# mengcaopku/DCNet

Hardware: AMD Instinct MI355X
Metric: clips/sec (T=8, 416x416, bs8) fwd+bwd (higher is better)
Workload: dtype f32; 1 GPU; T=8 416x416 bs8/GPU L=20 fp32, 64 img/GPU/step as pairs, fwd+5 losses+bwd+RMSprop; arith=f16x2-split MFMA, fp32 accumulate, parallelism=dp1, ranks_seen=1, reducer=none, step=hipGraph replay (fwd+losses+bwd+RMSprop), sampler=mt

## Files before the change

### dcnet_amd/csrc/conv3.hip

```cpp
#include "igemm.h"
#include "prof.h"
#include <type_traits>

namespace {

typedef _Float16 f16x8_t __attribute__((ext_vector_type(8)));
typedef _Float16 f16x4_t __attribute__((ext_vector_type(4)));
constexpr unsigned OOB3 = 0x80000000u;

__device__ __forceinline__ f32x4 ld16(__amdgpu_buffer_rsrc_t r, unsigned voff, unsigned soff) {
  return __builtin_bit_cast(f32x4, __builtin_amdgcn_raw_buffer_load_b128(r, voff, soff, 0));
}
__device__ __forceinline__ __amdgpu_buffer_rsrc_t rsrc3(const float* base, long long bytes) {
  const unsigned n = bytes > 0x7FFFFFF0LL ? 0x7FFFFFF0u : (bytes < 0 ? 0u : (unsigned)bytes);
  return __builtin_amdgcn_make_buffer_rsrc((void*)base, 0, n, 0x00020000);
}
__device__ __forceinline__ float pow2_scale3(unsigned amax_bits) {
  const int be = (int)((amax_bits >> 23) & 0xFF);
  if (be == 0 || be == 255) return 1.f;
  int e = 14 - (be - 126);
  e = e > 100 ? 100 : (e < -100 ? -100 : e);
  return __uint_as_float((unsigned)(e + 127) << 23);
}
__device__ __forceinline__ int row32(int pos, int half) { return pos * 32 + (((half ^ (pos >> 3)) & 1) << 4); }
// ... 430 lines not shown
#pragma unroll
    for (int r = 0; r < 16; ++r) {
      const int m = m0 + wm * 64 + mi * 32 + (r & 3) + 8 * (r >> 2) + 4 * half;
      if (m >= M) continue;
#pragma unroll
      for (int ni = 0; ni < 2; ++ni) {
        if (co_[ni] >= p.Co) continue;
        float v = acc[mi][ni][r] * sc[ni] + sh2[ni];
        if (p.act == DCN_ACT_LEAKY) v = v > 0.f ? v : v * p.slope;
        if (p.residual) v += p.residual[(size_t)m * p.ldr + co_[ni]];
        gout[(size_t)m * p.ldo + co_[ni]] = v;
        vmax = fmaxf(vmax, fabsf(v));
      }
    }
  if (p.amax_out) {
    vmax = wave_max(vmax);
    if (lane == 0) amax_update(p.amax_out, vmax, blockIdx.x * (WM * WN) + wave);
  }
}

DCN_KNOB(g_conv3, "3x3strip", 1, "conv3.hip: 3x3 stride-1 layers on the strip kernel (0 = implicit-GEMM tile)");
DCN_KNOB(g_conv3_bm, "3bm", 0, "conv3.hip: force the strip kernel's M tile (128 | 256; 0 = automatic)");
DCN_KNOB(g_conv3_abl, "3abl", 0, "conv3.hip: timing ablations of the strip kernel, bits (results WRONG)", nullptr, "-DC3_ABL=1", C3_ABL != 0);
DCN_KNOB(g_conv3_m16, "3m16", 1, "conv3.hip: conv3x.hip (16x16x32 MFMAs) for the launches that take the 256-row tile (0 = never; 2 = every strip launch it fits)");

template <int WM, int WN, int A_LD, int NP = 2, int ABL = 0, int LS = 0, bool IN16 = false, bool O32 = false>
int launch3(const IgemmParams& p, int gran, hipStream_t stream) {
  constexpr int NT = 64 * WM * WN, BM = 64 * WM, BN = 64 * WN;
  const int S = BM + 2 * p.Wi + 2;
  const size_t lds = (size_t)2 * NP * (S + 2) * 32 + (size_t)2 * 3 * (NP * BN * 32 + 128);
  static DcnPerDeviceFlag attr_once;
  if (attr_once.first()) {
    (void)hipFuncSetAttribute(reinterpret_cast<const void*>(&conv3_kernel<WM, WN, A_LD, NP, ABL, LS, IN16, O32>), hipFuncAttributeMaxDynamicSharedMemorySize, 160 * 1024);
  }
  const int gm = cdiv(p.M, BM), gn = cdiv(p.Co, BN);
  const double k_alg = 9.0 * p.Ci;
  const double alg_bytes = IN16 ? 2.0 * ((double)p.N * p.Hi * p.Wi * p.Ci + (double)p.Co * k_alg) +
                                      ((O32 ? 4.0 : 2.0) * (1.0 + (p.accumulate ? 1.0 : 0.0)) + (p.residual ? 2.0 : 0.0) + (p.bt_y ? 2.0 : 0.0)) * (double)p.M * p.Co
                                : 4.0 * ((double)p.N * p.Hi * p.Wi * p.Ci + (double)p.Co * k_alg + (double)p.M * p.Co * epilogue_reads(p));
  const int pid = prof_begin(IN16 ? 50 : (NP == 1 ? 33 : (WM == 4 ? 28 : 29)), 2.0 * (double)p.M * p.Co * k_alg, stream, alg_bytes);
  hipLaunchKernelGGL((conv3_kernel<WM, WN, A_LD, NP, ABL, LS, IN16, O32>), dim3(gm * gn), dim3(NT), lds, stream, p, S, gran);
  prof_end(pid, stream);
  DCN_CHECK_LAUNCH("conv3");
  return DCN_OK;
}

constexpr int A_LD_MAX = 4;
// ... 74 lines not shown
  }
  if (seen != 0x1FF) return false;
  const int bm = conv3b_bm(p.M, p.Co, p.Wi);
  if (!bm) return false;
  const int S = bm + 2 * p.Wi + 2;
  return (long long)S * p.ldi * 2 < 0x7FFFFFF0LL && (long long)p.Co * p.ldw * 2 < 0x7FFFFFF0LL;
}
int conv3b_launch(const IgemmParams& p0, int out_f32, hipStream_t stream) {
  IgemmParams p = p0;
  p.wt16 = p0.wt;
  const int bm = conv3b_bm(p.M, p.Co, p.Wi);
  const int S = bm + 2 * p.Wi + 2, need = cdiv(2 * S, 2 * bm);
  if (bm == 128) {
    if (need <= 2) return out_f32 ? launch3<2, 2, 2, 1, 0, 1, true, true>(p, bm, stream) : launch3<2, 2, 2, 1, 0, 1, true, false>(p, bm, stream);
    return out_f32 ? launch3<2, 2, 4, 1, 0, 1, true, true>(p, bm, stream) : launch3<2, 2, 4, 1, 0, 1, true, false>(p, bm, stream);
  }
  if (need <= 2) return out_f32 ? launch3<4, 2, 2, 1, 0, 1, true, true>(p, bm, stream) : launch3<4, 2, 2, 1, 0, 1, true, false>(p, bm, stream);
  return out_f32 ? launch3<4, 2, 4, 1, 0, 1, true, true>(p, bm, stream) : launch3<4, 2, 4, 1, 0, 1, true, false>(p, bm, stream);
}

int conv3_launch(const IgemmParams& p, int gran, hipStream_t stream) {
  int a_need; const int wmm = conv3_tile(p, gran, &a_need);
  if (g_conv3_m16 && !g_conv3_abl && conv3x_takes(p, gran)) {
    const long long wgs = (long long)cdiv(p.M, 256) * cdiv(p.Co, 128);
    const int cus = dcn_device_cus() > 0 ? dcn_device_cus() : 256;
    const bool short_tail = wgs > cus && wgs <= cus + cus / 2;
    if (g_conv3_m16 == 2 || !short_tail) return conv3x_launch(p, gran, stream);
  }
  if (wmm == 2) return launch3_ld<2, 2>(p, gran, stream);
  return launch3_ld<4, 2>(p, gran, stream);
}
```

### dcnet_amd/csrc/conv3x.hip

```cpp
#include "igemm.h"
#include "prof.h"
#include <type_traits>

namespace {

typedef _Float16 f16x8_t __attribute__((ext_vector_type(8)));
typedef _Float16 f16x4_t __attribute__((ext_vector_type(4)));
constexpr unsigned OOBX = 0x80000000u;

constexpr int XBM = 256, XBN = 128, XNT = 512, XWM = 4;
constexpr int XPB = XBN * 32;
constexpr int XPB1 = XPB + 64;
constexpr int XSLOT = 2 * XPB + 128;
constexpr int XSTAGE = 6 * XSLOT;
constexpr int XA_LD = 4;
#ifndef C3X_ABL
#define C3X_ABL 0
#endif
constexpr int XSMAX = 466;
constexpr int XPA = (XSMAX + 2) * 32;

__device__ __forceinline__ f32x4 ldx16(__amdgpu_buffer_rsrc_t r, unsigned voff, unsigned soff) {
  return __builtin_bit_cast(f32x4, __builtin_amdgcn_raw_buffer_load_b128(r, voff, soff, 0));
}
__device__ __forceinline__ __amdgpu_buffer_rsrc_t rsrcx(const float* base, long long bytes) {
  const unsigned n = bytes > 0x7FFFFFF0LL ? 0x7FFFFFF0u : (bytes < 0 ? 0u : (unsigned)bytes);
  return __builtin_amdgcn_make_buffer_rsrc((void*)base, 0, n, 0x00020000);
}
__device__ __forceinline__ float pow2_scalex(unsigned amax_bits) {
  const int be = (int)((amax_bits >> 23) & 0xFF);
  if (be == 0 || be == 255) return 1.f;
  int e = 14 - (be - 126);
  e = e > 100 ? 100 : (e < -100 ? -100 : e);
  return __uint_as_float((unsigned)(e + 127) << 23);
}

typedef __attribute__((address_space(3))) void lds_voidx;
template <bool DMA>
__global__ __launch_bounds__(XNT, 2) void conv3x_kernel(const IgemmParams p, const int S, const int gran) {
  extern __shared__ __attribute__((aligned(16))) unsigned char smemx[];
  constexpr int PA = XPA;
  unsigned char* const Abase = smemx;
  unsigned char* const Bbase = smemx + 4 * PA;

  const int tid = threadIdx.x, lane = tid & 63, wave = tid >> 6;
  const int wm = wave >> 1, wn = wave & 1;
  const int c16 = lane & 15, g = lane >> 4, tsel = g >> 1, half = g & 1;
  const int gn = (p.Co + XBN - 1) / XBN;
  const int lin = xcd_remap(blockIdx.x, gridDim.x);
  const int bm = lin / gn, bn = lin - bm * gn;
  const int W = p.Wi, H = p.Hi, M = p.M;
  const int m0 = bm * XBM;
  const float sa = pow2_scalex(amax_read(p.amax_a)), sb = p.b_scale[0];

  const int lin0 = m0 - W - 1;
  const int base_px = lin0 > 0 ? lin0 : 0;
  const float* a_base = p.in + (long long)base_px * p.ldi;
  const __amdgpu_buffer_rsrc_t a_rs = rsrcx(a_base, ((long long)(M - base_px - 1) * p.ldi + p.Ci) * 4);
  const __amdgpu_buffer_rsrc_t b_rs = rsrcx(p.wt, (long long)p.Co * p.ldw * 4);

  const int pos0 = tid >> 2, q0 = tid & 3;
  const unsigned a_off0 = (unsigned)((lin0 + pos0 - base_px) * p.ldi * 4 + q0 * 16);
  const int a_st0 = pos0 * 32 + q0 * 8;
  const unsigned a_pstride = (unsigned)(128 * p.ldi * 4);
// ... 8 lines not shown
    unsigned o = a_off0;
    asm volatile("" : "+v"(o));
    return a_ok[j] ? o + (unsigned)j * a_pstride : OOBX;
  };
  auto a_st = [&](const int j) {
    int o = a_st0;
    asm volatile("" : "+v"(o));
    return a_in[j] ? o + j * 4096 : (XSMAX + 1) * 32 + q0 * 8;
  };
  unsigned b_off; int b_st;
  if constexpr (DMA) {
    const int plane = wave & 1, rho = 32 * (wave >> 1) + (lane >> 1), kh = lane & 1;
    const int filt = (rho & ~63) + 4 * (rho & 15) + ((rho & 63) >> 4);
    const int co = bn * XBN + filt;
    b_off = co < p.Co ? (unsigned)(co * p.ldw * 4 + (2 * kh + plane) * 16) : OOBX;
    b_st = __builtin_amdgcn_readfirstlane(plane * XPB1 + (wave >> 1) * 1024);
  } else {
    const int rho = tid >> 2, chunk = tid & 3;
    const int filt = (rho & ~63) + 4 * (rho & 15) + ((rho & 63) >> 4);
    const int co = bn * XBN + filt;
    b_off = co < p.Co ? (unsigned)(co * p.ldw * 4 + chunk * 16) : OOBX;
    b_st = (chunk & 1) * XPB1 + rho * 32 + (chunk >> 1) * 16;
  }
  unsigned msk[4];
#pragma unroll
  for (int i = 0; i < 4; ++i) {
    const int m = m0 + wm * 64 + i * 16 + c16;
    unsigned v = 0;
    if (m < M) {
      const int rem = m % (H * W), y = rem / W, x = rem - y * W;
      for (int t = 0; t < 9; ++t)
        if ((unsigned)(y + p.tap_dy[t]) < (unsigned)H && (unsigned)(x + p.tap_dx[t]) < (unsigned)W) v |= 1u << t;
    }
    msk[i] = v;
  }
  const int a_lane0 = (wm * 64 + c16) * 32 + half * 16;
  const int b_lane0 = (wn * 64 + c16) * 32 + half * 16 + tsel * 3 * XSLOT;

  const int nch = p.Ci >> 4;
  const int nper = nch >> 1;
  const int nsi = 3 * nper;

  f32x4 a_reg[XA_LD], b_reg[6];
  const unsigned lds0 = (unsigned)(uintptr_t)(lds_voidx*)smemx;
  auto store_a_piece = [&](const int buf_off, int j) {
    const f32x4 t = a_reg[j] * sa;
    const f16x4_t h = {(_Float16)t[0], (_Float16)t[1], (_Float16)t[2], (_Float16)t[3]};
    const f16x4_t l = {(_Float16)(t[0] - (float)h[0]), (_Float16)(t[1] - (float)h[1]), (_Float16)(t[2] - (float)h[2]),
                       (_Float16)(t[3] - (float)h[3])};
    if constexpr (DMA) {
      const unsigned addr = lds0 + (unsigned)(buf_off + a_st(j));
      asm volatile("ds_write_b64 %0, %1\n\tds_write_b64 %0, %2 offset:%3"
                   :: "v"(addr), "v"(__builtin_bit_cast(unsigned long long, h)), "v"(__builtin_bit_cast(unsigned long long, l)), "n"(XPA));
    } else {
      unsigned char* abuf = Abase + buf_off;
      *reinterpret_cast<uint2*>(abuf + a_st(j)) = __builtin_bit_cast(uint2, h);
      *reinterpret_cast<uint2*>(abuf + PA + a_st(j)) = __builtin_bit_cast(uint2, l);
    }
  };

  f32x4 acc[4][4];
#pragma unroll
  for (int i = 0; i < 4; ++i)
#pragma unroll
    for (int j = 0; j < 4; ++j) acc[i][j] = f32x4{0.f, 0.f, 0.f, 0.f};

  if (tid < 8) {
    const f32x4 z = {0.f, 0.f, 0.f, 0.f};
    *reinterpret_cast<f32x4*>(Abase + (tid >> 1) * PA + XSMAX * 32 + (tid & 1) * 16) = z;
  }
#pragma unroll
  for (int j = 0; j < XA_LD; ++j) a_reg[j] = ldx16(a_rs, a_off(j), 0u);
  auto dma = [&](const int stage_off, const int slot, const bool live, const unsigned soff) {
    __builtin_amdgcn_raw_ptr_buffer_load_lds(b_rs, (lds_voidx*)(Bbase + stage_off + slot * XSLOT + b_st), 16, (int)(live ? b_off : OOBX),
                                             (int)(live ? soff : 0u), 0, 0);
  };
  if constexpr (DMA) {
#pragma unroll
    for (int q = 0; q < 6; ++q) {
      const int G = q / 3, j = q - 3 * G;
      dma(0, q, true, (unsigned)p.tap_w[3 * G + j] * 4u);
    }
#pragma unroll
    for (int q = 0; q < 2; ++q)
      dma(XSTAGE, q, true, (unsigned)p.tap_w[6 + q] * 4u);
#pragma unroll
// ... 1 lines not shown
#pragma unroll
    for (int j = 0; j < XA_LD; ++j) a_reg[j] = ldx16(a_rs, a_off(j), 64u);
    asm volatile("s_waitcnt vmcnt(0)" ::: "memory");
  } else {
#pragma unroll
    for (int q = 0; q < 6; ++q) {
      const int G = q / 3, j = q - 3 * G;
      b_reg[q] = ldx16(b_rs, b_off, (unsigned)p.tap_w[3 * G + j] * 4u);
    }
#pragma unroll
    for (int j = 0; j < XA_LD; ++j) store_a_piece(0, j);
#pragma unroll
    for (int j = 0; j < XA_LD; ++j) a_reg[j] = ldx16(a_rs, a_off(j), 64u);
#pragma unroll
    for (int q = 0; q < 6; ++q) *reinterpret_cast<f32x4*>(Bbase + q * XSLOT + b_st) = b_reg[q];
#pragma unroll
    for (int q = 0; q < 6; ++q) {
      const int G = q < 3 ? 2 : 0, cc = q < 3 ? 0 : 1, j = q % 3;
      b_reg[q] = ldx16(b_rs, b_off, (unsigned)(p.tap_w[3 * G + j] + cc * 16) * 4u);
    }
  }
  __syncthreads();

  f16x8_t Al[4], Ah[4], Bh[4], Bl[4];
  int ad[4];
  auto a_addr = [&](const int T, const int J) {
    const int Ga = T == 0 ? 0 : (T == 1 ? 2 : 1), Gb = T == 0 ? 1 : (T == 1 ? 0 : 2);
    const int ta = 3 * Ga + J, tb = 3 * Gb + J;
    const int sha = (p.tap_dy[ta] + 1) * W + p.tap_dx[ta] + 1, shb = (p.tap_dy[tb] + 1) * W + p.tap_dx[tb] + 1;
    int ts = tsel;
    asm volatile("" : "+v"(ts));
    const int sh = ts ? shb : sha;
    const int tl = ts ? tb : ta;
    const int bo = T == 0 ? 0 : (T == 2 ? 2 * PA : ts * (2 * PA));
    const int base = bo + a_lane0 + sh * 32;
    const int z = bo + XSMAX * 32;
#pragma unroll
    for (int i = 0; i < 4; ++i) ad[i] = ((msk[i] >> tl) & 1) ? base + i * 512 : z;
  };
  auto read_Al = [&]() {
#pragma unroll
    for (int i = 0; i < 4; ++i) Al[i] = *reinterpret_cast<const f16x8_t*>(Abase + PA + ad[i]);
  };
  auto read_Ah = [&]() {
#pragma unroll
    for (int i = 0; i < 4; ++i) Ah[i] = *reinterpret_cast<const f16x8_t*>(Abase + ad[i]);
  };
  int st_cur = 0;
  auto read_B = [&](f16x8_t (&B)[4], const int stage_off, const int J, const int plane) {
    const unsigned char* bb = Bbase + stage_off + b_lane0;
#pragma unroll
    for (int jn = 0; jn < 4; ++jn) B[jn] = *reinterpret_cast<const f16x8_t*>(bb + J * XSLOT + plane * XPB1 + jn * 512);
  };
  auto mm = [&](const f16x8_t (&A)[4], const f16x8_t (&B)[4]) {
#pragma unroll
    for (int i = 0; i < 4; ++i)
#pragma unroll
      for (int jn = 0; jn < 4; ++jn) acc[i][jn] = __builtin_amdgcn_mfma_f32_16x16x32_f16(A[i], B[jn], acc[i][jn], 0, 0, 0);
  };

  auto body = [&](auto T_, const int u) {
    constexpr int T = decltype(T_)::value;
    constexpr int TN = (T + 1) % 3;
    const int k = 3 * u + T, c0 = 2 * u;
    const bool in_b = k + 2 < nsi;
    const int st_nxt = XSTAGE - st_cur;
    unsigned char* const bw = Bbase + st_nxt + b_st;
    auto side = [&](const int gi) {
      if constexpr (DMA) {
        if (gi < 4 && !(C3X_ABL & 1)) {
          const int sl = gi + 2, second = sl >= 3, j = sl - 3 * second;
          const int G = T == 0 ? (second ? 0 : 2) : (T == 1 ? (second ? 2 : 1) : (second ? 1 : 0));
          const int dc = T == 0 ? (second ? 1 : 0) : (T == 1 ? 1 : 2);
          dma(st_nxt, sl, k + 1 < nsi, (unsigned)(p.tap_w[3 * G + j] + (c0 + dc) * 16) * 4u);
        }
        if (gi >= 7 && !(C3X_ABL & 1)) {
          const int sl = gi - 7;
          const int G = T == 0 ? 1 : (T == 1 ? 0 : 2), dc = T == 0 ? 1 : 2;
          dma(st_cur, sl, in_b, (unsigned)(p.tap_w[3 * G + sl] + (c0 + dc) * 16) * 4u);
// ... 41 lines not shown
      mm(Ah, Bh);
      side(3 * j + 1);
      __builtin_amdgcn_sched_barrier(0);
      if (j < 2) read_B(Bh, st_cur, j + 1, 0); else read_B(Bh, st_nxt, 0, 0);
      __builtin_amdgcn_sched_barrier(0);
      mm(Ah, Bl);
      side(3 * j + 2);
      __builtin_amdgcn_sched_barrier(0);
    }
    st_cur = st_nxt;
  };
  a_addr(0, 0);
  read_Al();
  read_B(Bh, 0, 0, 0);
  {
    using I0 = std::integral_constant<int, 0>; using I1 = std::integral_constant<int, 1>; using I2 = std::integral_constant<int, 2>;
    for (int u = 0; u < nper; ++u) { body(I0{}, u); body(I1{}, u); body(I2{}, u); }
  }
  if constexpr (DMA) asm volatile("s_waitcnt vmcnt(0)" ::: "memory");
  __syncthreads();

  const float dq = 1.f / (sa * sb);
#pragma unroll
  for (int i = 0; i < 4; ++i)
#pragma unroll
    for (int jn = 0; jn < 4; ++jn) acc[i][jn] *= dq;
  const int co0 = bn * XBN + wn * 64 + 4 * c16;
  const bool co_ok = co0 < p.Co;
  const int mrow0 = m0 + wm * 64 + 4 * g;
  float* __restrict__ gout = p.out;
  if (p.accumulate && co_ok) {
#pragma unroll
    for (int i = 0; i < 4; ++i)
#pragma unroll
      for (int r = 0; r < 4; ++r) {
        const int m = mrow0 + 16 * i + r;
        if (m >= M) continue;
        const f32x4 o = *reinterpret_cast<const f32x4*>(gout + (size_t)m * p.ldo + co0);
#pragma unroll
        for (int jn = 0; jn < 4; ++jn) acc[i][jn][r] += o[jn];
      }
  }
  if (p.stats) {
    float* red = reinterpret_cast<float*>(smemx);
    float s[4] = {0.f, 0.f, 0.f, 0.f}, ss[4] = {0.f, 0.f, 0.f, 0.f};
    if (p.bt_y && co_ok) {
      const f32x4 mu = *reinterpret_cast<const f32x4*>(p.bt_mean + co0), is = *reinterpret_cast<const f32x4*>(p.bt_invstd + co0);
      f32x4 ga = {1.f, 1.f, 1.f, 1.f}, be = {0.f, 0.f, 0.f, 0.f};
      if (p.bt_gamma) ga = *reinterpret_cast<const f32x4*>(p.bt_gamma + co0);
      if (p.bt_beta) be = *reinterpret_cast<const f32x4*>(p.bt_beta + co0);
      const float* yb = p.bt_y + co0;
#pragma unroll
      for (int i = 0; i < 4; ++i) {
        f32x4 yv[4];
#pragma unroll
        for (int r = 0; r < 4; ++r) {
          const int m = mrow0 + 16 * i + r;
          yv[r] = *reinterpret_cast<const f32x4*>(yb + (size_t)(m < M ? m : M - 1) * p.Co);
        }
#pragma unroll
        for (int r = 0; r < 4; ++r) {
          const int m = mrow0 + 16 * i + r;
#pragma unroll
          for (int jn = 0; jn < 4; ++jn) {
            const float xh = (yv[r][jn] - mu[jn]) * is[jn];
            float gq = acc[i][jn][r];
            if (p.bt_act == DCN_ACT_LEAKY) gq = (ga[jn] * xh + be[jn] <= 0.f) ? gq * p.bt_slope : gq;
            gq = m < M ? gq : 0.f;
            s[jn] += gq; ss[jn] += gq * xh;
          }
        }
      }
    } else if (!p.bt_y) {
#pragma unroll
      for (int i = 0; i < 4; ++i)
#pragma unroll
        for (int r = 0; r < 4; ++r)
#pragma unroll
          for (int jn = 0; jn < 4; ++jn) { const float v = acc[i][jn][r]; s[jn] += v; ss[jn] = __builtin_fmaf(v, v, ss[jn]); }
    }
#pragma unroll
    for (int jn = 0; jn < 4; ++jn) {
      s[jn] += __shfl_xor(s[jn], 16); ss[jn] += __shfl_xor(ss[jn], 16);
      s[jn] += __shfl_xor(s[jn], 32); ss[jn] += __shfl_xor(ss[jn], 32);
    }
    if (g == 0) {
      const int col = wn * 64 + 4 * c16;
      *reinterpret_cast<f32x4*>(red + (0 * XWM + wm) * XBN + col) = f32x4{s[0], s[1], s[2], s[3]};
      *reinterpret_cast<f32x4*>(red + (1 * XWM + wm) * XBN + col) = f32x4{ss[0], ss[1], ss[2], ss[3]};
    }
    __syncthreads();
    const int groups = XBM / gran, spg = XWM / groups;
    const int rows_total = (M + gran - 1) / gran;
    for (int idx = tid; idx < 2 * XBN * groups; idx += XNT) {
      const int gq = idx / (2 * XBN), rest = idx - gq * 2 * XBN;
      const int which = rest / XBN, col = rest - which * XBN;
      float t = 0.f;
      for (int w = 0; w < spg; ++w) t += red[(which * XWM + gq * spg + w) * XBN + col];
      const int co = bn * XBN + col, srow = bm * groups + gq;
      if (co < p.Co && srow < rows_total) p.stats[((size_t)srow * 2 + which) * p.Co + co] = t;
    }
  }
  float vmax = 0.f;
  if (co_ok) {
    f32x4 sc = {1.f, 1.f, 1.f, 1.f}, sh = {0.f, 0.f, 0.f, 0.f};
    if (p.scale) sc = *reinterpret_cast<const f32x4*>(p.scale + co0);
    if (p.shift) sh = *reinterpret_cast<const f32x4*>(p.shift + co0);
#pragma unroll
    for (int i = 0; i < 4; ++i)
#pragma unroll
      for (int r = 0; r < 4; ++r) {
        const int m = mrow0 + 16 * i + r;
        if (m >= M) continue;
        f32x4 v;
#pragma unroll
        for (int jn = 0; jn < 4; ++jn) {
          float t = acc[i][jn][r] * sc[jn] + sh[jn];
          if (p.act == DCN_ACT_LEAKY) t = t > 0.f ? t : t * p.slope;
          v[jn] = t;
        }
        if (p.residual) v += *reinterpret_cast<const f32x4*>(p.residual + (size_t)m * p.ldr + co0);
        *reinterpret_cast<f32x4*>(gout + (size_t)m * p.ldo + co0) = v;
#pragma unroll
        for (int jn = 0; jn < 4; ++jn) vmax = fmaxf(vmax, fabsf(v[jn]));
      }
  }
  if (p.amax_out) {
    vmax = wave_max(vmax);
    if (lane == 0) amax_update(p.amax_out, vmax, blockIdx.x * 8 + wave);
  }
}

}

bool conv3x_takes(const IgemmParams& p, int gran) {
  if (p.wt16 || (gran != 128 && gran != 256)) return false;
  if (p.Co % 4 != 0 || p.ldo % 4 != 0 || (p.residual && p.ldr % 4 != 0)) return false;
  auto al16 = [](const void* q) { return (reinterpret_cast<uintptr_t>(q) & 15) == 0; };
  if (!al16(p.out) || !al16(p.residual) || !al16(p.bt_y) || !al16(p.scale) || !al16(p.shift) || !al16(p.bt_mean) || !al16(p.bt_invstd) ||
      !al16(p.bt_gamma) || !al16(p.bt_beta)) return false;
  const int S = XBM + 2 * p.Wi + 2;
  if (S > XSMAX) return false;
  return (long long)S * p.ldi * 4 < 0x7FFFFFF0LL && (long long)p.Co * p.ldw * 4 < 0x7FFFFFF0LL;
}

int conv3x_launch(const IgemmParams& p, int gran, hipStream_t stream) {
  const int S = XBM + 2 * p.Wi + 2;
  const size_t lds = (size_t)4 * XPA + (size_t)2 * XSTAGE;
  static_assert((size_t)4 * XPA + (size_t)2 * XSTAGE <= 160 * 1024, "LDS");
  static DcnPerDeviceFlag attr_once;
  if (attr_once.first()) {
    (void)hipFuncSetAttribute(reinterpret_cast<const void*>(&conv3x_kernel<true>), hipFuncAttributeMaxDynamicSharedMemorySize, 160 * 1024);
  }
  const int gm = cdiv(p.M, XBM), gn = cdiv(p.Co, XBN);
  const double k_alg = 9.0 * p.Ci;
  const double alg_bytes = 4.0 * ((double)p.N * p.Hi * p.Wi * p.Ci + (double)p.Co * k_alg + (double)p.M * p.Co * epilogue_reads(p));
  const int pid = prof_begin(51, 2.0 * (double)p.M * p.Co * k_alg, stream, alg_bytes);
  hipLaunchKernelGGL(conv3x_kernel<true>, dim3(gm * gn), dim3(XNT), lds, stream, p, S, gran);
  prof_end(pid, stream);
  DCN_CHECK_LAUNCH("conv3x");
  return DCN_OK;
}
```

### dcnet_amd/csrc/igemm.h

```cpp
#pragma once
#include "common.h"

#define IGEMM_MAX_TAPS 16


struct IgemmParams {
  const float* in;
  const float* wt;
  const float* f8;
  const unsigned* amax_a;
  const unsigned* amax_b;
  const void* wt16;
  const float* b_scale;
  unsigned* amax_out;
  float* out;
  const float* scale;
  const float* shift;
  const float* residual;
  float* stats;
  const float* row_scale;
  int batch;
  long long in_bs, wt_bs, out_bs;
  int bmode;
  int kvalid;
// ... 5 lines not shown
  int Co, ldo, ldr, ldw;
  int M;
  int ntaps;
  int cpt, kiters;
  int act; float slope;
  int accumulate, dense_out, c4;
  int acc_post;
  int tap_dy[IGEMM_MAX_TAPS], tap_dx[IGEMM_MAX_TAPS], tap_w[IGEMM_MAX_TAPS];
  int ncls;
  int cls_M[4], cls_Hs[4], cls_Ws[4], cls_oy0[4], cls_ox0[4], cls_ntaps[4];
  const float* bt_y; const float* bt_mean; const float* bt_invstd; const float* bt_gamma; const float* bt_beta;
  int bt_act; float bt_slope;
  const unsigned char* a_scale8; const unsigned char* b_scale8;
};
inline double epilogue_reads(const IgemmParams& p) { return 1.0 + (p.accumulate ? 1.0 : 0.0) + (p.residual ? 1.0 : 0.0) + (p.bt_y ? 1.0 : 0.0); }
bool igemm_tap_capable(const IgemmParams& p);

int igemm_grid_m(int M, int Co, int ntaps);
int igemm_launch(const IgemmParams& p, hipStream_t stream);
bool igemm_will_presplit(long long rows, int Co, int ntaps, int Ci);

bool conv3_applicable(const IgemmParams& p, int precision, int gran);
int conv3_launch(const IgemmParams& p, int gran, hipStream_t stream);
bool conv3x_takes(const IgemmParams& p, int gran);
int conv3x_launch(const IgemmParams& p, int gran, hipStream_t stream);
int conv3b_bm(int M, int Co, int Wi);
bool conv3b_takes(const IgemmParams& p);
int conv3b_launch(const IgemmParams& p, int out_f32, hipStream_t stream);

bool conv1_applicable(const IgemmParams& p, int precision, int gran);
int conv1_launch(const IgemmParams& p, int gran, hipStream_t stream);
int conv1_tile_of(long long rows, int Co, int ntaps, int Ci, int stats, int gran, int storage16);
int conv1b_grid_m(int M, int Co, int ntaps, int s1_w = 0);
int conv1b_launch(const IgemmParams& p, int out_f32, hipStream_t stream);
int conv1q_grid_m(int M, int Co);
int conv1q_launch(const IgemmParams& p, int out_f32, hipStream_t stream);
bool conv2b_takes(int M, int Co, int ntaps);
int conv2b_launch(const IgemmParams& p, int out_f32, hipStream_t stream);


bool stem_applicable(const IgemmParams& p, const float* scratch);
int stem_launch(const IgemmParams& p, float* scratch, hipStream_t stream);

bool dgrad2_applicable(int n, int h, int wd, int cin, int cout, int ksize, int stride, int accumulate);
struct DcnBnTap { const float* y; const float* mean; const float* invstd; const float* gamma; const float* beta; int act; float slope;
                  float* stats; int stats_rows; };
int nconv1_launch_b16(int mode, const void* x, int ldi, const void* w16, void* y, int ldo, float* stats, int stats_rows,
                      int n, int h, int wd, int stride, hipStream_t stream);
// ... 19 lines not shown
```

### dcnet_amd/lib.py

```python
from __future__ import annotations

import ctypes
import os
from ctypes import c_char_p, c_double, c_float, c_int, c_int64, c_void_p

_HERE = os.path.dirname(os.path.abspath(__file__))
LIB_PATH = os.path.join(_HERE, "libdcnet_hip.so")

P, I, L, F, D = c_void_p, c_int, c_int64, c_float, c_double

SIGNATURES = {
    "dcn_last_error": (c_char_p, []),
    "dcn_version": (I, []),
    "dcn_nchw_to_nhwc": (I, [P, P, I, I, I, I, I, P]),
    "dcn_nhwc_to_nchw": (I, [P, P, I, I, I, I, I, P]),
    "dcn_oihw_to_ohwi": (I, [P, P, I, I, I, I, I, P]),
    "dcn_ohwi_to_oihw": (I, [P, P, I, I, I, I, I, P]),
    "dcn_conv2d_fwd": (I, [P, P, P, I, I, I, I, I, I, I, P, P, I, F, P, I, I, P, I, P, P, P, P, P, I, P]),
    "dcn_absmax": (I, [P, L, I, I, P, P]),
    "dcn_f8_scale": (I, [P, L, I, I, P, P, P]),
    "dcn_conv2d_stats_rows": (I, [I, I, I, I, I, I]),
    "dcn_conv1_tile": (I, [L, I, I, I, I, I]),
    "dcn_l2norm_score_fwd_form": (I, [I]),
    "dcn_bn_apply_form": (I, [I, I]),
    "dcn_igemm_split_build": (I, [I, I]),
    "dcn_gemm3_variant": (I, []),
    "dcn_conv2d_bwd_data": (I, [P, I, P, P, P, I, I, I, I, I, I, I, I, P, P, P, I, P, P]),
    "dcn_conv2d_bwd_data_tap": (I, [P, I, P, P, P, I, I, I, I, I, I, I, I, P, P, P, I, P, P, P, P, P, P, I, F, P, I, P, P]),
    "dcn_conv2d_bwd_data_tap_rows": (I, [I, I, I, I, I, I, I]),
    "dcn_conv2d_pre_supported": (I, [I, I, I, I, I, I, I]),
    "dcn_conv2d_fwd_pre": (I, [P, P, P, I, I, I, I, I, I, I, P, P, I, F, I, P, P, P, P]),
    "dcn_conv2d_bwd_weight_pre_supported": (I, [I, I, I, I, I, I, I]),
    "dcn_conv2d_bwd_weight_pre": (I, [P, I, P, I, P, P, P, I, I, I, I, I, I, I, P, P, I, F, P, P, P]),
    "dcn_bn_act_amax_bound": (I, [P, P, P, I, F, P, P]),
    "dcn_gemm3_supported": (I, [I, I, I, I]),
    "dcn_gemm3_presplit": (I, [P, I, L, P, I, L, I, I, I, P, P]),
    "dcn_gemm3": (I, [P, I, L, I, P, I, L, I, P, I, L, P, L, I, I, I, I, I, P, P, P]),
    "dcn_filter_job_bytes": (I, []),
    "dcn_prepare_filters": (I, [P, I, I, I, P, L, P]),
    "dcn_conv2d_geom_size": (L, [I, I, I, I, I]),
    "dcn_conv2d_geom": (I, [P, I, I, I, I, I, P]),
    "dcn_conv2d_bwd_weight": (I, [P, I, P, I, P, P, P, P, I, I, I, I, I, I, I, P, P, P]),
    "dcn_conv2d_bwd_weight_ws": (L, [I, I, I, I, I, I, I]),
    "dcn_stem_bwd_weight_bn": (I, [P, P, P, I, P, P, P, P, I, F, P, L, I, I, I, I, P, P, P]),
    "dcn_stem_bwd_weight_bn_ws": (L, [I, I, I]),
    "dcn_stem_bwd_weight_bn_b16": (I, [P, P, P, I, P, P, P, P, I, F, P, L, I, I, I, I, P, P, P]),
    "dcn_bn_ws": (L, [I]),
    "dcn_bn_finalize": (I, [P, I, I, L, P, P, F, F, P, P, P, P, P, P, P, P]),
    "dcn_bn_fold": (I, [P, P, P, P, F, I, P, P, P]),
# ... 131 lines not shown
    "dcn_conv2d_fwd_f8": (I, [P, P, P, P, P, I, I, I, I, I, I, I, I, P, P, I, F, P, I, I, P, I, P]),
    "dcn_conv2d_bwd_data_f8": (I, [P, P, P, P, P, I, I, I, I, I, I, I, I, I, P, P, P, P, P, I, F, P, I, P, P]),
    "dcn_post_topk": (I, [P, P, P, P, P, I, I, I, I, P, P, P, P, P, P, P, P, P]),
    "dcn_post_fusion": (I, [P, P, P, P, I, I, I, I, P, P, P]),
    "dcn_clip_prep_ws": (L, [I, I]),
    "dcn_clip_prep": (I, [P, L, P, P, I, I, P, P, P, P]),
    "dcn_bank_write": (I, [P, I, P, P, L, I, P]),
    "dcn_coattn_bank_fwd": (I, [P, P, P, P, L, P, P, I, L, P, P, P, P, I, I, I, F, P]),
    "dcn_post_fusion_bank": (I, [P, P, I, I, I, I, P, P, P]),
    "dcn_bank_write_b16": (I, [P, I, P, P, P, L, I, P]),
    "dcn_bank_concat_b16": (I, [P, L, P, I, L, P, I, I, I, P]),
    "dcn_coattn_bank_form": (I, [I, I]),
    "dcn_post_nms": (I, [P, I, I, F, P, P]),
    "dcn_tube_transitions": (I, [P, P, I, I, I, I, I, I, F, F, P, P]),
    "dcn_tube_forward": (I, [P, P, P, P, I, I, I, I, I, P, P, P]),
    "dcn_tube_backtrack": (I, [P, P, I, I, I, P, P, P]),
    "dcn_tube_stream_step": (I, [P, P, P, I, I, I, I, I, P, P, P, P, P]),
    "dcn_tube_stream_flush": (I, [P, P, I, I, I, I, P, P, P]),
}
_VALUE_FUNCS = {"dcn_version", "dcn_conv2d_stats_rows", "dcn_conv2d_bwd_data_tap_rows", "dcn_conv2d_pre_supported",
                "dcn_conv2d_bwd_weight_pre_supported", "dcn_gemm3_supported", "dcn_channel_stats_rows", "dcn_filter_job_bytes", "dcn_prof_records",
                "dcn_conv2d_stats_rows_b16", "dcn_bn_act_bwd_reduce_rows_b16", "dcn_conv2d_stats_rows_f8", "dcn_quant_fusable", "dcn_quant_job_bytes",
                "dcn_conv1_tile", "dcn_l2norm_score_fwd_form", "dcn_bn_apply_form", "dcn_igemm_split_build", "dcn_gemm3_variant",
                "dcn_coattn_bank_form"}
ABI_VERSION = 318


class DcnError(RuntimeError):
    pass


class _Lib:
    def __init__(self, path: str):
        if not os.path.exists(path):
            raise DcnError(
                f"{path} not found: build it with `python -m dcnet_amd.build` "
                "(hipcc --offload-arch=gfx950).  There is no CPU or eager fallback.")
        self._dll = ctypes.CDLL(path)
        for name, (res, args) in SIGNATURES.items():
            try:
                fn = getattr(self._dll, name)
            except AttributeError as e:
                raise DcnError(f"{path} does not export {name}; rebuild the library") from e
            fn.restype = res
            fn.argtypes = args
            if res is I and name not in _VALUE_FUNCS:
                setattr(self, name[4:], self._checked(name, fn))
# ... 41 lines not shown
```

### include/dcnet_hip.h

```cpp
#ifndef DCNET_HIP_H
#define DCNET_HIP_H

#include <stdint.h>

#ifdef __cplusplus
extern "C" {
#endif

#define DCN_OK 0
#define DCN_ERR_ARG (-1)
#define DCN_ERR_LAUNCH (-2)

#define DCN_AMAX_WORDS 64
#define DCN_SLAB_COUNTERS 4096

#define DCN_ACT_NONE 0
#define DCN_ACT_LEAKY 1

#define DCN_ABI_VERSION 318

const char* dcn_last_error(void);
int dcn_version(void);

int dcn_nchw_to_nhwc(const float* src, float* dst, int n, int c, int h, int w, int c_pad, void* stream);
int dcn_nhwc_to_nchw(const float* src, float* dst, int n, int c, int h, int w, int ld, void* stream);
int dcn_oihw_to_ohwi(const float* src, float* dst, int co, int ci, int kh, int kw, int ci_pad, void* stream);
int dcn_ohwi_to_oihw(const float* src, float* dst, int co, int ci, int kh, int kw, int ci_pad, void* stream);

int dcn_conv2d_fwd(const float* x, const float* w, float* y,
                   int n, int h, int wd, int cin, int cout, int ksize, int stride,
                   const float* scale, const float* shift, int act, float slope,
                   const float* residual, int ldr, int ldy,
                   float* stats, int accumulate, const float* f8_scales,
                   const uint32_t* amax_x, const uint32_t* amax_w, uint32_t* amax_y, float* w_split, int w_split_ready,
                   void* stream);
int dcn_absmax(const float* x, int64_t rows, int c, int ld, uint32_t* amax, void* stream);
int dcn_conv2d_stats_rows(int n, int h, int wd, int cout, int ksize, int stride);
int dcn_conv1_tile(int64_t rows, int cout, int ntaps, int cin, int stats, int storage);
int dcn_l2norm_score_fwd_form(int c);
int dcn_bn_apply_form(int c, int params_aligned);
int dcn_igemm_split_build(int kind, int ksteps);
int dcn_gemm3_variant(void);
int dcn_f8_scale(const float* x, int64_t rows, int c, int ld, float* scale, void* ws, void* stream);

int dcn_conv2d_bwd_data(const float* dy, int lddy, const float* w, float* wt, float* dx,
                        int n, int h, int wd, int cin, int cout, int ksize, int stride,
                        int accumulate, const float* f8_scales, const uint32_t* amax_dy, const uint32_t* amax_w,
                        int wt_ready, const float* wt_split, void* stream);
int dcn_conv2d_bwd_data_tap(const float* dy, int lddy, const float* w, float* wt, float* dx,
                            int n, int h, int wd, int cin, int cout, int ksize, int stride,
                            int accumulate, const float* f8_scales, const uint32_t* amax_dy, const uint32_t* amax_w,
                            int wt_ready, const float* wt_split,
                            const float* tap_y, const float* tap_mean, const float* tap_invstd, const float* tap_gamma,
                            const float* tap_beta, int tap_act, float tap_slope, float* tap_stats, int tap_stats_rows,
                            int* tap_rows, void* stream);
int dcn_conv2d_bwd_data_tap_rows(int n, int h, int wd, int cin, int cout, int ksize, int stride);
int dcn_conv2d_pre_supported(int n, int h, int wd, int cin, int cout, int ksize, int stride);
int dcn_conv2d_fwd_pre(const float* x, const float* w, float* y, int n, int h, int wd, int cin, int cout, int ksize, int stride,
                       const float* pre_scale, const float* pre_shift, int pre_act, float pre_slope,
                       int ldy, float* stats, const uint32_t* amax_x, const uint32_t* amax_w, void* stream);
int dcn_conv2d_bwd_weight_pre_supported(int n, int h, int wd, int cin, int cout, int ksize, int stride);
int dcn_conv2d_bwd_weight_pre(const float* x, int ldx, const float* dy, int lddy, float* dw, float* ws, uint32_t* counters,
                              int n, int h, int wd, int cin, int cout, int ksize, int stride,
                              const float* pre_scale, const float* pre_shift, int pre_act, float pre_slope,
                              const uint32_t* amax_x, const uint32_t* amax_dy, void* stream);
// ... 353 lines not shown
```

Measured before the change: 88.49 clips/s.

## Add 128/192-row tile variants to conv3x and pick tile height by wave quantization

The 16x16x32-MFMA strip kernel is templated on the M tile height (128, 192 or 256 rows), and a cost table picks the height that minimizes rounds of workgroups over the CU count. Grids that previously fell back to the older strip kernel on a short tail can now run conv3x with a smaller tile that fills the last round better. Statistics partials are restricted to tile heights that map onto the slab granularity, and the 128-row tile chains its per-wave sums through LDS. The cost weights are heuristic, so a smaller tile may lose per-tile reuse without gaining enough occupancy.

Result: no change. 88.40 clips/s (-0.1%).

```diff
diff --git a/dcnet_amd/csrc/conv3.hip b/dcnet_amd/csrc/conv3.hip
--- a/dcnet_amd/csrc/conv3.hip
+++ b/dcnet_amd/csrc/conv3.hip
@@ -476,7 +476,7 @@
 DCN_KNOB(g_conv3, "3x3strip", 1, "conv3.hip: 3x3 stride-1 layers on the strip kernel (0 = implicit-GEMM tile)");
 DCN_KNOB(g_conv3_bm, "3bm", 0, "conv3.hip: force the strip kernel's M tile (128 | 256; 0 = automatic)");
 DCN_KNOB(g_conv3_abl, "3abl", 0, "conv3.hip: timing ablations of the strip kernel, bits (results WRONG)", nullptr, "-DC3_ABL=1", C3_ABL != 0);
-DCN_KNOB(g_conv3_m16, "3m16", 1, "conv3.hip: conv3x.hip (16x16x32 MFMAs) for the launches that take the 256-row tile (0 = never; 2 = every strip launch it fits)");
+DCN_KNOB(g_conv3_m16, "3m16", 1, "conv3.hip: conv3x.hip (16x16x32 MFMAs; 1 = 256-row tiles, 192-row tiles where conv3x_pick_bm says so, other grids of 1 to 1.5 rounds of 256-row tiles on conv3.hip; 0 = never; 2 = every strip launch it fits, at that height; 3 = 256-row tiles only, the rule before the tile heights; 128 | 192 | 256 = that tile height forced where the launch's partial rows admit it)");
 
 template <int WM, int WN, int A_LD, int NP = 2, int ABL = 0, int LS = 0, bool IN16 = false, bool O32 = false>
 int launch3(const IgemmParams& p, int gran, hipStream_t stream) {
@@ -597,10 +597,15 @@
 int conv3_launch(const IgemmParams& p, int gran, hipStream_t stream) {
   int a_need; const int wmm = conv3_tile(p, gran, &a_need);
   if (g_conv3_m16 && !g_conv3_abl && conv3x_takes(p, gran)) {
+    const int cus = dcn_device_cus() > 0 ? dcn_device_cus() : 256;
+    const int flags = conv3x_flags(p, gran);
     const long long wgs = (long long)cdiv(p.M, 256) * cdiv(p.Co, 128);
-    const int cus = dcn_device_cus() > 0 ? dcn_device_cus() : 256;
     const bool short_tail = wgs > cus && wgs <= cus + cus / 2;
-    if (g_conv3_m16 == 2 || !short_tail) return conv3x_launch(p, gran, stream);
+    if (g_conv3_m16 == 128 || g_conv3_m16 == 192 || g_conv3_m16 == 256) return conv3x_launch(p, gran, conv3x_fit_bm(g_conv3_m16, flags), stream);
+    const int bm = g_conv3_m16 == 3 ? 256 : conv3x_pick_bm(p.M, p.Co, p.Wi, cus, flags);
+    if (g_conv3_m16 == 2) return conv3x_launch(p, gran, bm, stream);
+    if (bm == 192) return conv3x_launch(p, gran, 192, stream);
+    if (!short_tail) return conv3x_launch(p, gran, 256, stream);
   }
   if (wmm == 2) return launch3_ld<2, 2>(p, gran, stream);
   return launch3_ld<4, 2>(p, gran, stream);
diff --git a/dcnet_amd/csrc/conv3x.hip b/dcnet_amd/csrc/conv3x.hip
--- a/dcnet_amd/csrc/conv3x.hip
+++ b/dcnet_amd/csrc/conv3x.hip
@@ -8,17 +8,21 @@
 typedef _Float16 f16x4_t __attribute__((ext_vector_type(4)));
 constexpr unsigned OOBX = 0x80000000u;
 
-constexpr int XBM = 256, XBN = 128, XNT = 512, XWM = 4;
+constexpr int XBN = 128, XNT = 512, XWM = 4;
+static_assert(XBN == 128 && CONV3X_WMAX == 104, "igemm.h");
+template <int MI> struct XTile {
+  static constexpr int BM = 64 * MI;
+  static constexpr int SMAX = BM + 2 * CONV3X_WMAX + 2;
+  static constexpr int PA = (SMAX + 2) * 32;
+  static constexpr int A_LD = (SMAX + 127) / 128;
+};
 constexpr int XPB = XBN * 32;
 constexpr int XPB1 = XPB + 64;
 constexpr int XSLOT = 2 * XPB + 128;
 constexpr int XSTAGE = 6 * XSLOT;
-constexpr int XA_LD = 4;
 #ifndef C3X_ABL
 #define C3X_ABL 0
 #endif
-constexpr int XSMAX = 466;
-constexpr int XPA = (XSMAX + 2) * 32;
 
 __device__ __forceinline__ f32x4 ldx16(__amdgpu_buffer_rsrc_t r, unsigned voff, unsigned soff) {
   return __builtin_bit_cast(f32x4, __builtin_amdgcn_raw_buffer_load_b128(r, voff, soff, 0));
@@ -36,10 +40,10 @@
 }
 
 typedef __attribute__((address_space(3))) void lds_voidx;
-template <bool DMA>
+template <bool DMA, int MI>
 __global__ __launch_bounds__(XNT, 2) void conv3x_kernel(const IgemmParams p, const int S, const int gran) {
   extern __shared__ __attribute__((aligned(16))) unsigned char smemx[];
-  constexpr int PA = XPA;
+  constexpr int XBM = XTile<MI>::BM, XSMAX = XTile<MI>::SMAX, XPA = XTile<MI>::PA, XA_LD = XTile<MI>::A_LD, PA = XPA;
   unsigned char* const Abase = smemx;
   unsigned char* const Bbase = smemx + 4 * PA;
 
@@ -94,10 +98,10 @@
     b_off = co < p.Co ? (unsigned)(co * p.ldw * 4 + chunk * 16) : OOBX;
     b_st = (chunk & 1) * XPB1 + rho * 32 + (chunk >> 1) * 16;
   }
-  unsigned msk[4];
-#pragma unroll
-  for (int i = 0; i < 4; ++i) {
-    const int m = m0 + wm * 64 + i * 16 + c16;
+  unsigned msk[MI];
+#pragma unroll
+  for (int i = 0; i < MI; ++i) {
+    const int m = m0 + wm * (16 * MI) + i * 16 + c16;
     unsigned v = 0;
     if (m < M) {
       const int rem = m % (H * W), y = rem / W, x = rem - y * W;
@@ -106,7 +110,7 @@
     }
     msk[i] = v;
   }
-  const int a_lane0 = (wm * 64 + c16) * 32 + half * 16;
+  const int a_lane0 = (wm * (16 * MI) + c16) * 32 + half * 16;
   const int b_lane0 = (wn * 64 + c16) * 32 + half * 16 + tsel * 3 * XSLOT;
 
   const int nch = p.Ci >> 4;
@@ -131,9 +135,9 @@
     }
   };
 
-  f32x4 acc[4][4];
-#pragma unroll
-  for (int i = 0; i < 4; ++i)
+  f32x4 acc[MI][4];
+#pragma unroll
+  for (int i = 0; i < MI; ++i)
 #pragma unroll
     for (int j = 0; j < 4; ++j) acc[i][j] = f32x4{0.f, 0.f, 0.f, 0.f};
 
@@ -181,8 +185,8 @@
   }
   __syncthreads();
 
-  f16x8_t Al[4], Ah[4], Bh[4], Bl[4];
-  int ad[4];
+  f16x8_t Al[MI], Ah[MI], Bh[4], Bl[4];
+  int ad[MI];
   auto a_addr = [&](const int T, const int J) {
     const int Ga = T == 0 ? 0 : (T == 1 ? 2 : 1), Gb = T == 0 ? 1 : (T == 1 ? 0 : 2);
     const int ta = 3 * Ga + J, tb = 3 * Gb + J;
@@ -195,15 +199,15 @@
     const int base = bo + a_lane0 + sh * 32;
     const int z = bo + XSMAX * 32;
 #pragma unroll
-    for (int i = 0; i < 4; ++i) ad[i] = ((msk[i] >> tl) & 1) ? base + i * 512 : z;
+    for (int i = 0; i < MI; ++i) ad[i] = ((msk[i] >> tl) & 1) ? base + i * 512 : z;
   };
   auto read_Al = [&]() {
 #pragma unroll
-    for (int i = 0; i < 4; ++i) Al[i] = *reinterpret_cast<const f16x8_t*>(Abase + PA + ad[i]);
+    for (int i = 0; i < MI; ++i) Al[i] = *reinterpret_cast<const f16x8_t*>(Abase + PA + ad[i]);
   };
   auto read_Ah = [&]() {
 #pragma unroll
-    for (int i = 0; i < 4; ++i) Ah[i] = *reinterpret_cast<const f16x8_t*>(Abase + ad[i]);
+    for (int i = 0; i < MI; ++i) Ah[i] = *reinterpret_cast<const f16x8_t*>(Abase + ad[i]);
   };
   int st_cur = 0;
   auto read_B = [&](f16x8_t (&B)[4], const int stage_off, const int J, const int plane) {
@@ -211,9 +215,9 @@
 #pragma unroll
     for (int jn = 0; jn < 4; ++jn) B[jn] = *reinterpret_cast<const f16x8_t*>(bb + J * XSLOT + plane * XPB1 + jn * 512);
   };
-  auto mm = [&](const f16x8_t (&A)[4], const f16x8_t (&B)[4]) {
-#pragma unroll
-    for (int i = 0; i < 4; ++i)
+  auto mm = [&](const f16x8_t (&A)[MI], const f16x8_t (&B)[4]) {
+#pragma unroll
+    for (int i = 0; i < MI; ++i)
 #pragma unroll
       for (int jn = 0; jn < 4; ++jn) acc[i][jn] = __builtin_amdgcn_mfma_f32_16x16x32_f16(A[i], B[jn], acc[i][jn], 0, 0, 0);
   };
@@ -301,16 +305,16 @@
 
   const float dq = 1.f / (sa * sb);
 #pragma unroll
-  for (int i = 0; i < 4; ++i)
+  for (int i = 0; i < MI; ++i)
 #pragma unroll
     for (int jn = 0; jn < 4; ++jn) acc[i][jn] *= dq;
   const int co0 = bn * XBN + wn * 64 + 4 * c16;
   const bool co_ok = co0 < p.Co;
-  const int mrow0 = m0 + wm * 64 + 4 * g;
+  const int mrow0 = m0 + wm * (16 * MI) + 4 * g;
   float* __restrict__ gout = p.out;
   if (p.accumulate && co_ok) {
 #pragma unroll
-    for (int i = 0; i < 4; ++i)
+    for (int i = 0; i < MI; ++i)
 #pragma unroll
       for (int r = 0; r < 4; ++r) {
         const int m = mrow0 + 16 * i + r;
@@ -320,17 +324,17 @@
         for (int jn = 0; jn < 4; ++jn) acc[i][jn][r] += o[jn];
       }
   }
-  if (p.stats) {
+  if constexpr (MI != 3) if (p.stats) {
     float* red = reinterpret_cast<float*>(smemx);
     float s[4] = {0.f, 0.f, 0.f, 0.f}, ss[4] = {0.f, 0.f, 0.f, 0.f};
-    if (p.bt_y && co_ok) {
+    if (MI == 4 && p.bt_y && co_ok) {
       const f32x4 mu = *reinterpret_cast<const f32x4*>(p.bt_mean + co0), is = *reinterpret_cast<const f32x4*>(p.bt_invstd + co0);
       f32x4 ga = {1.f, 1.f, 1.f, 1.f}, be = {0.f, 0.f, 0.f, 0.f};
       if (p.bt_gamma) ga = *reinterpret_cast<const f32x4*>(p.bt_gamma + co0);
       if (p.bt_beta) be = *reinterpret_cast<const f32x4*>(p.bt_beta + co0);
       const float* yb = p.bt_y + co0;
 #pragma unroll
-      for (int i = 0; i < 4; ++i) {
+      for (int i = 0; i < MI; ++i) {
         f32x4 yv[4];
 #pragma unroll
         for (int r = 0; r < 4; ++r) {
@@ -351,25 +355,45 @@
         }
       }
     } else if (!p.bt_y) {
-#pragma unroll
-      for (int i = 0; i < 4; ++i)
-#pragma unroll
-        for (int r = 0; r < 4; ++r)
-#pragma unroll
-          for (int jn = 0; jn < 4; ++jn) { const float v = acc[i][jn][r]; s[jn] += v; ss[jn] = __builtin_fmaf(v, v, ss[jn]); }
+      auto fold = [&]() {
+#pragma unroll
+        for (int i = 0; i < MI; ++i)
+#pragma unroll
+          for (int r = 0; r < 4; ++r)
+#pragma unroll
+            for (int jn = 0; jn < 4; ++jn) { const float v = acc[i][jn][r]; s[jn] += v; ss[jn] = __builtin_fmaf(v, v, ss[jn]); }
+      };
+      if constexpr (MI == 2) {
+        f32x4* chain = reinterpret_cast<f32x4*>(smemx + 2 * XWM * XBN * 4) + (((wm >> 1) * 2 + wn) * 64 + lane) * 2;
+        if (!(wm & 1)) {
+          fold();
+          chain[0] = f32x4{s[0], s[1], s[2], s[3]}; chain[1] = f32x4{ss[0], ss[1], ss[2], ss[3]};
+        }
+        __syncthreads();
+        if (wm & 1) {
+          const f32x4 s0 = chain[0], ss0 = chain[1];
+#pragma unroll
+          for (int jn = 0; jn < 4; ++jn) { s[jn] = s0[jn]; ss[jn] = ss0[jn]; }
+          fold();
+        }
+      } else {
+        fold();
+      }
     }
 #pragma unroll
     for (int jn = 0; jn < 4; ++jn) {
       s[jn] += __shfl_xor(s[jn], 16); ss[jn] += __shfl_xor(ss[jn], 16);
       s[jn] += __shfl_xor(s[jn], 32); ss[jn] += __shfl_xor(ss[jn], 32);
     }
-    if (g == 0) {
+    constexpr int NSL = XBM / 64;
+    const int slab = MI == 2 ? wm >> 1 : wm;
+    if (g == 0 && (MI != 2 || (wm & 1))) {
       const int col = wn * 64 + 4 * c16;
-      *reinterpret_cast<f32x4*>(red + (0 * XWM + wm) * XBN + col) = f32x4{s[0], s[1], s[2], s[3]};
-      *reinterpret_cast<f32x4*>(red + (1 * XWM + wm) * XBN + col) = f32x4{ss[0], ss[1], ss[2], ss[3]};
+      *reinterpret_cast<f32x4*>(red + (0 * XWM + slab) * XBN + col) = f32x4{s[0], s[1], s[2], s[3]};
+      *reinterpret_cast<f32x4*>(red + (1 * XWM + slab) * XBN + col) = f32x4{ss[0], ss[1], ss[2], ss[3]};
     }
     __syncthreads();
-    const int groups = XBM / gran, spg = XWM / groups;
+    const int groups = XBM / gran, spg = NSL / groups;
     const int rows_total = (M + gran - 1) / gran;
     for (int idx = tid; idx < 2 * XBN * groups; idx += XNT) {
       const int gq = idx / (2 * XBN), rest = idx - gq * 2 * XBN;
@@ -386,7 +410,7 @@
     if (p.scale) sc = *reinterpret_cast<const f32x4*>(p.scale + co0);
     if (p.shift) sh = *reinterpret_cast<const f32x4*>(p.shift + co0);
 #pragma unroll
-    for (int i = 0; i < 4; ++i)
+    for (int i = 0; i < MI; ++i)
 #pragma unroll
       for (int r = 0; r < 4; ++r) {
         const int m = mrow0 + 16 * i + r;
@@ -418,25 +442,66 @@
   auto al16 = [](const void* q) { return (reinterpret_cast<uintptr_t>(q) & 15) == 0; };
   if (!al16(p.out) || !al16(p.residual) || !al16(p.bt_y) || !al16(p.scale) || !al16(p.shift) || !al16(p.bt_mean) || !al16(p.bt_invstd) ||
       !al16(p.bt_gamma) || !al16(p.bt_beta)) return false;
-  const int S = XBM + 2 * p.Wi + 2;
-  if (S > XSMAX) return false;
+  if (p.Wi > CONV3X_WMAX) return false;
+  const int S = 256 + 2 * p.Wi + 2;
   return (long long)S * p.ldi * 4 < 0x7FFFFFF0LL && (long long)p.Co * p.ldw * 4 < 0x7FFFFFF0LL;
 }
 
-int conv3x_launch(const IgemmParams& p, int gran, hipStream_t stream) {
-  const int S = XBM + 2 * p.Wi + 2;
-  const size_t lds = (size_t)4 * XPA + (size_t)2 * XSTAGE;
-  static_assert((size_t)4 * XPA + (size_t)2 * XSTAGE <= 160 * 1024, "LDS");
+static const struct { int bm; double cost; } CONV3X_COST[] = {{256, 1.0}, {192, 0.82}, {128, 0.61}};
+
+static bool conv3x_bm_ok(int bm, int flags) {
+  if (!(flags & CONV3X_PARTIALS)) return true;
+  return bm == 256 || (bm == 128 && !(flags & (CONV3X_PARTIALS_256 | CONV3X_TAP)));
+}
+
+int conv3x_pick_bm(int M, int Co, int Wi, int num_cus, int flags) {
+  if (M <= 0 || Co <= 0 || Wi > CONV3X_WMAX) return 0;
+  if (num_cus <= 0) num_cus = 256;
+  const long long gn = cdiv(Co, XBN);
+  int best = 0; double best_t = 0.0;
+  for (const auto& c : CONV3X_COST) {
+    if (!conv3x_bm_ok(c.bm, flags)) continue;
+    const double t = (double)cdiv((long long)cdiv(M, c.bm) * gn, (long long)num_cus) * c.cost;
+    if (!best || t < best_t) { best = c.bm; best_t = t; }
+  }
+  return best;
+}
+int conv3x_fit_bm(int bm, int flags) {
+  if (bm == 192 && !conv3x_bm_ok(192, flags)) bm = 128;
+  if (bm == 128 && !conv3x_bm_ok(128, flags)) bm = 256;
+  return bm == 128 || bm == 192 ? bm : 256;
+}
+
+namespace {
+template <int MI>
+int launch3x(const IgemmParams& p, int gran, hipStream_t stream) {
+  using T = XTile<MI>;
+  const int S = T::BM + 2 * p.Wi + 2;
+  constexpr size_t lds = (size_t)4 * T::PA + (size_t)2 * XSTAGE;
+  static_assert(lds <= 160 * 1024, "LDS");
+  static_assert(2 * XWM * XBN * 4 + 2 * 2 * 64 * 2 * 16 <= lds, "statistics reduction in LDS");
+  static_assert(T::A_LD <= 4 && T::A_LD * 128 >= T::SMAX, "strip pieces");
   static DcnPerDeviceFlag attr_once;
   if (attr_once.first()) {
-    (void)hipFuncSetAttribute(reinterpret_cast<const void*>(&conv3x_kernel<true>), hipFuncAttributeMaxDynamicSharedMemorySize, 160 * 1024);
-  }
-  const int gm = cdiv(p.M, XBM), gn = cdiv(p.Co, XBN);
+    (void)hipFuncSetAttribute(reinterpret_cast<const void*>(&conv3x_kernel<true, MI>), hipFuncAttributeMaxDynamicSharedMemorySize, 160 * 1024);
+  }
+  const int gm = cdiv(p.M, T::BM), gn = cdiv(p.Co, XBN);
   const double k_alg = 9.0 * p.Ci;
   const double alg_bytes = 4.0 * ((double)p.N * p.Hi * p.Wi * p.Ci + (double)p.Co * k_alg + (double)p.M * p.Co * epilogue_reads(p));
   const int pid = prof_begin(51, 2.0 * (double)p.M * p.Co * k_alg, stream, alg_bytes);
-  hipLaunchKernelGGL(conv3x_kernel<true>, dim3(gm * gn), dim3(XNT), lds, stream, p, S, gran);
+  hipLaunchKernelGGL((conv3x_kernel<true, MI>), dim3(gm * gn), dim3(XNT), lds, stream, p, S, gran);
   prof_end(pid, stream);
   DCN_CHECK_LAUNCH("conv3x");
   return DCN_OK;
 }
+}
+
+int conv3x_launch(const IgemmParams& p, int gran, int bm, hipStream_t stream) {
+  DCN_CHECK_ARG(conv3x_bm_ok(bm, conv3x_flags(p, gran)) && p.Wi <= CONV3X_WMAX, "conv3x: a %d-row tile cannot write this launch's partial rows", bm);
+  if (bm == 128) return launch3x<2>(p, gran, stream);
+  if (bm == 192) return launch3x<3>(p, gran, stream);
+  DCN_CHECK_ARG(bm == 256, "conv3x: tile height %d", bm);
+  return launch3x<4>(p, gran, stream);
+}
+
+extern "C" int dcn_conv3x_pick_bm(int m, int cout, int wi, int num_cus, int flags) { return conv3x_pick_bm(m, cout, wi, num_cus, flags); }
diff --git a/dcnet_amd/csrc/igemm.h b/dcnet_amd/csrc/igemm.h
--- a/dcnet_amd/csrc/igemm.h
+++ b/dcnet_amd/csrc/igemm.h
@@ -51,8 +51,15 @@
 
 bool conv3_applicable(const IgemmParams& p, int precision, int gran);
 int conv3_launch(const IgemmParams& p, int gran, hipStream_t stream);
+constexpr int CONV3X_WMAX = 104;
+enum { CONV3X_PARTIALS = 1, CONV3X_PARTIALS_256 = 2, CONV3X_TAP = 4 };
+inline int conv3x_flags(const IgemmParams& p, int gran) {
+  return p.stats ? CONV3X_PARTIALS | (gran == 256 ? CONV3X_PARTIALS_256 : 0) | (p.bt_y ? CONV3X_TAP : 0) : 0;
+}
 bool conv3x_takes(const IgemmParams& p, int gran);
-int conv3x_launch(const IgemmParams& p, int gran, hipStream_t stream);
+int conv3x_pick_bm(int M, int Co, int Wi, int num_cus, int flags);
+int conv3x_fit_bm(int bm, int flags);
+int conv3x_launch(const IgemmParams& p, int gran, int bm, hipStream_t stream);
 int conv3b_bm(int M, int Co, int Wi);
 bool conv3b_takes(const IgemmParams& p);
 int conv3b_launch(const IgemmParams& p, int out_f32, hipStream_t stream);
diff --git a/dcnet_amd/lib.py b/dcnet_amd/lib.py
--- a/dcnet_amd/lib.py
+++ b/dcnet_amd/lib.py
@@ -25,6 +25,7 @@
     "dcn_bn_apply_form": (I, [I, I]),
     "dcn_igemm_split_build": (I, [I, I]),
     "dcn_gemm3_variant": (I, []),
+    "dcn_conv3x_pick_bm": (I, [I, I, I, I, I]),
     "dcn_conv2d_bwd_data": (I, [P, I, P, P, P, I, I, I, I, I, I, I, I, P, P, P, I, P, P]),
     "dcn_conv2d_bwd_data_tap": (I, [P, I, P, P, P, I, I, I, I, I, I, I, I, P, P, P, I, P, P, P, P, P, P, I, F, P, I, P, P]),
     "dcn_conv2d_bwd_data_tap_rows": (I, [I, I, I, I, I, I, I]),
@@ -202,7 +203,7 @@
                 "dcn_conv2d_bwd_weight_pre_supported", "dcn_gemm3_supported", "dcn_channel_stats_rows", "dcn_filter_job_bytes", "dcn_prof_records",
                 "dcn_conv2d_stats_rows_b16", "dcn_bn_act_bwd_reduce_rows_b16", "dcn_conv2d_stats_rows_f8", "dcn_quant_fusable", "dcn_quant_job_bytes",
                 "dcn_conv1_tile", "dcn_l2norm_score_fwd_form", "dcn_bn_apply_form", "dcn_igemm_split_build", "dcn_gemm3_variant",
-                "dcn_coattn_bank_form"}
+                "dcn_coattn_bank_form", "dcn_conv3x_pick_bm"}
 ABI_VERSION = 318
 
 
diff --git a/include/dcnet_hip.h b/include/dcnet_hip.h
--- a/include/dcnet_hip.h
+++ b/include/dcnet_hip.h
@@ -41,6 +41,7 @@
 int dcn_bn_apply_form(int c, int params_aligned);
 int dcn_igemm_split_build(int kind, int ksteps);
 int dcn_gemm3_variant(void);
+int dcn_conv3x_pick_bm(int m, int cout, int wi, int num_cus, int flags);
 int dcn_f8_scale(const float* x, int64_t rows, int c, int ld, float* scale, void* ws, void* stream);
 
 int dcn_conv2d_bwd_data(const float* dy, int lddy, const float* w, float* wt, float* dx,
```
